# Hfx-J/SGTD

Measured on AMD Instinct MI355X. Metric: query frames/sec vs map size (descriptor build + candidate selection), higher is better.
Workload: dtype f64

## Files before the change

sgtd_amd/csrc/build_kernel.hip.h:

```cpp
#pragma once
#include "common.hip.h"

struct DescArrays {
  double *side, *angle, *center;
  float *vertex;
  int *label;
  u32 *frame;
  int *node_id;
  QueryRec *qrec;
};

#define SGTD_BUILD_THREADS 1024
#ifdef SGTD_EXP_PHASE
__device__ unsigned long long g_bphase[8];
#define BPH(i) do { if (tid == 0) { const unsigned long long _n = __builtin_readcyclecounter(); atomicAdd(&g_bphase[i], _n - bph_t); bph_t = _n; } } while (0)
#else
#define BPH(i) do { } while (0)
#endif
#define SGTD_TRI_INVALID 0xFFFFFFFFFFFFFFFFull
#define SGTD_SLOT_EMPTY 0xFFFFFFFFu

struct Tri {
  double a, b, c;
  int va, vb, vc;
  bool valid;
};

__device__ __forceinline__ double side_len(const float4 &p, const float4 &q) {
  double dx = (double)(p.x - q.x), dy = (double)(p.y - q.y), dz = (double)(p.z - q.z);
  return sqrt(dx * dx + dy * dy + dz * dz);
}

__device__ __forceinline__ Tri make_triangle(const float4 &p1, const float4 &p2,
                                             const float4 &p3, const DevCfg &cfg) {
  Tri t;
  double a = side_len(p1, p2), b = side_len(p1, p3), c = side_len(p3, p2);
  t.valid = !(a > cfg.max_len || b > cfg.max_len || c > cfg.max_len ||
              a < cfg.min_len || b < cfg.min_len || c < cfg.min_len);
  int sa = 0, sb = 1, sc = 2;
  double tmp; int ti;
  if (a > b) { tmp = a; a = b; b = tmp; ti = sa; sa = sb; sb = ti; }
  if (b > c) { tmp = b; b = c; c = tmp; ti = sb; sb = sc; sc = ti; }
  if (a > b) { tmp = a; a = b; b = tmp; ti = sa; sa = sb; sb = ti; }
  t.a = a; t.b = b; t.c = c;
  t.va = sa + sb - 1;
  t.vb = sa + sc - 1;
  t.vc = sb + sc - 1;
  return t;
}

__host__ __device__ __forceinline__ u64 pack_milli_key(u64 x, u64 y, u64 z) { return (x << 42) | (y << 21) | z; }
__device__ __forceinline__ u64 milli_key(const Tri &t) {
  float kx = (float)(t.a * 1000.0), ky = (float)(t.b * 1000.0), kz = (float)(t.c * 1000.0);
  u64 x = (u64)(long long)kx, y = (u64)(long long)ky, z = (u64)(long long)kz;
  return pack_milli_key(x, y, z);
}

struct BuildParams {
  const float *xyz;
  const u32 *label;
  const long long *kp_off;
  int n_frames;
  u32 frame_id0;
  int frame_id_step;
  long long out_stride;
  u32 *out_count;
  int max_n;
  int max_slots;
  u64 *ws_keys;
  u32 *ws_slots;
};

template <bool LDS_DEDUP, int KM>
__global__ __launch_bounds__(SGTD_BUILD_THREADS) void build_frames_kernel(
    BuildParams P, DevCfg cfg, DescArrays out) {
  extern __shared__ __align__(16) unsigned char smem[];
  const int K = cfg.K, tpi = cfg.tpi;
  const int max_t = P.max_n * tpi;
  const int max_words = (max_t + 31) / 32;
  float4 *pts = reinterpret_cast<float4 *>(smem);
  size_t off = (size_t)P.max_n * 16;
  unsigned short *knn = reinterpret_cast<unsigned short *>(smem + off);
  off += (((size_t)P.max_n * K * 2) + 15) & ~(size_t)15;
  unsigned char *mn = smem + off;
  off += (((size_t)tpi * 2) + 15) & ~(size_t)15;
  u32 *winbits = reinterpret_cast<u32 *>(smem + off);
  off += (((size_t)max_words * 4) + 15) & ~(size_t)15;
  u32 *wordpre = reinterpret_cast<u32 *>(smem + off);
  off += (((size_t)(max_words + 1) * 4) + 15) & ~(size_t)15;
  u64 *keys;
  u32 *slots;
  if (LDS_DEDUP) {
    keys = reinterpret_cast<u64 *>(smem + off);
    off += (size_t)max_t * 8;
    slots = reinterpret_cast<u32 *>(smem + off);
  } else {
    keys = P.ws_keys + (size_t)blockIdx.x * max_t;
    slots = P.ws_slots + (size_t)blockIdx.x * P.max_slots;
  }
  const int tid = threadIdx.x;

  if (tid == 0) {
    int k = 0;
    for (int m = 1; m < K - 1; m++)
      for (int n = m + 1; n < K; n++) {
        mn[2 * k] = (unsigned char)m;
        mn[2 * k + 1] = (unsigned char)n;
        k++;
      }
  }

  for (int f = blockIdx.x; f < P.n_frames; f += gridDim.x) {
    const long long kp0 = P.kp_off[f];
    const int n = (int)(P.kp_off[f + 1] - kp0);
    __syncthreads();
    if (n < K) {
      if (tid == 0) P.out_count[f] = 0;
      continue;
    }
    const int T = n * tpi;
    int nslots = 64;
    while (nslots < T + 1) nslots <<= 1;
    const int nwords = (T + 31) / 32;

#ifdef SGTD_EXP_PHASE
    unsigned long long bph_t = __builtin_readcyclecounter();
#endif
    for (int i = tid; i < n; i += SGTD_BUILD_THREADS) {
      float4 p;
      p.x = P.xyz[(kp0 + i) * 3 + 0];
      p.y = P.xyz[(kp0 + i) * 3 + 1];
      p.z = P.xyz[(kp0 + i) * 3 + 2];
      p.w = __uint_as_float(P.label[kp0 + i]);
      pts[i] = p;
    }
    for (int s = tid; s < nslots; s += SGTD_BUILD_THREADS) slots[s] = SGTD_SLOT_EMPTY;
    for (int w = tid; w < nwords; w += SGTD_BUILD_THREADS) winbits[w] = 0;
    __syncthreads();

    BPH(0);
    const int parts = (3 * K <= tpi) ? 4 : 1;
    const int per_pass = SGTD_BUILD_THREADS / parts;
    for (int i0 = 0; i0 < n; i0 += per_pass) {
      const int i = i0 + tid / parts, part = tid % parts;
      float bd[KM];
      int bi[KM];
#pragma unroll
      for (int k = 0; k < KM; k++) { bd[k] = __builtin_inff(); bi[k] = 0; }
      auto insert = [&](float cd, int cj) {
        bool lt = false;
#pragma unroll
        for (int k = 0; k < KM; k++) {
          lt = lt || (cd < bd[k]);
          float td = lt ? bd[k] : cd; int tj = lt ? bi[k] : cj;
          bd[k] = lt ? cd : bd[k]; bi[k] = lt ? cj : bi[k];
          cd = td; cj = tj;
        }
      };
      if (i < n) {
        const float4 q = pts[i];
        const int j_lo = (int)((long long)n * part / parts), j_hi = (int)((long long)n * (part + 1) / parts);
        for (int j = j_lo; j < j_hi; j++) {
          const float4 p = pts[j];
          float dx = q.x - p.x, dy = q.y - p.y, dz = q.z - p.z;
          float d = dx * dx;
          d += dy * dy;
          d += dz * dz;
          insert(d, j);
        }
        if (part > 0) {
#pragma unroll
          for (int k = 0; k < KM; k++)
            if (k < K) keys[((size_t)i * 3 + (part - 1)) * K + k] = ((u64)__float_as_uint(bd[k]) << 32) | (u32)bi[k];
        }
      }
      if (parts > 1) {
        if (!LDS_DEDUP) __threadfence_block();
        __syncthreads();
        if (i < n && part == 0) {
          for (int pk = 0; pk < 3 * K; pk++) {
            const u64 v = keys[(size_t)i * 3 * K + pk];
            insert(__uint_as_float((u32)(v >> 32)), (int)(u32)v);
          }
        }
      }
      if (i < n && part == 0) {
#pragma unroll
        for (int k = 0; k < KM; k++)
          if (k < K) knn[i * K + k] = (unsigned short)bi[k];
      }
      if (parts > 1) __syncthreads();
    }
    __syncthreads();

    BPH(1);
    for (int t = tid; t < T; t += SGTD_BUILD_THREADS) {
      const int i = t / tpi, r = t - i * tpi;
      const int m = mn[2 * r], nn = mn[2 * r + 1];
      Tri tr = make_triangle(pts[i], pts[knn[i * K + m]], pts[knn[i * K + nn]], cfg);
      keys[t] = tr.valid ? milli_key(tr) : SGTD_TRI_INVALID;
    }
    if (!LDS_DEDUP) __threadfence_block();
    __syncthreads();

    BPH(2);
    for (int t = tid; t < T; t += SGTD_BUILD_THREADS) {
      const u64 key = keys[t];
      if (key == SGTD_TRI_INVALID) continue;
      u32 h = (u32)mix64(key) & (u32)(nslots - 1);
      while (true) {
        u32 cur = atomicCAS(&slots[h], SGTD_SLOT_EMPTY, (u32)t);
        if (cur == SGTD_SLOT_EMPTY) break;
        if (keys[cur] == key) { atomicMin(&slots[h], (u32)t); break; }
        h = (h + 1) & (u32)(nslots - 1);
      }
    }
    __syncthreads();
    for (int s = tid; s < nslots; s += SGTD_BUILD_THREADS) {
      u32 v = slots[s];
      if (v != SGTD_SLOT_EMPTY) atomicOr(&winbits[v >> 5], 1u << (v & 31));
    }
    __syncthreads();
    if (tid < SGTD_WAVE) {
      u32 carry = 0;
      for (int w0 = 0; w0 < nwords; w0 += SGTD_WAVE) {
        int w = w0 + tid;
        u32 c = (w < nwords) ? __popc(winbits[w]) : 0;
        u32 inc = wave_incl_scan(c);
        if (w < nwords) wordpre[w] = carry + inc - c;
        carry += __shfl(inc, SGTD_WAVE - 1);
      }
      if (tid == 0) { wordpre[nwords] = carry; P.out_count[f] = carry; }
    }
    __syncthreads();

    BPH(3);
    const u32 frame_id = P.frame_id0 + (u32)(P.frame_id_step * f);
    for (int t = tid; t < T; t += SGTD_BUILD_THREADS) {
      const u32 word = winbits[t >> 5];
      if (!((word >> (t & 31)) & 1u)) continue;
      const u32 rank = wordpre[t >> 5] + __popc(word & ((1u << (t & 31)) - 1u));
      const int i = t / tpi, r = t - i * tpi;
      const int m = mn[2 * r], nn = mn[2 * r + 1];
      float4 p[3];
      p[0] = pts[i]; p[1] = pts[knn[i * K + m]]; p[2] = pts[knn[i * K + nn]];
      const Tri tr = make_triangle(p[0], p[1], p[2], cfg);
      const float4 A = tr.va == 0 ? p[0] : (tr.va == 1 ? p[1] : p[2]);
      const float4 B = tr.vb == 0 ? p[0] : (tr.vb == 1 ? p[1] : p[2]);
      const float4 C = tr.vc == 0 ? p[0] : (tr.vc == 1 ? p[1] : p[2]);
      const size_t o = (size_t)f * P.out_stride + rank;
      const double a = tr.a, b = tr.b, c = tr.c;
      out.side[o * 3 + 0] = cfg.scale * a;
      out.side[o * 3 + 1] = cfg.scale * b;
      out.side[o * 3 + 2] = cfg.scale * c;
      out.angle[o * 3 + 0] = fabs((b * b + c * c - a * a) / (2 * b * c));
      out.angle[o * 3 + 1] = fabs((a * a + c * c - b * b) / (2 * a * c));
      out.angle[o * 3 + 2] = fabs((a * a + b * b - c * c) / (2 * a * b));
      out.center[o * 3 + 0] = (((double)A.x + (double)B.x) + (double)C.x) / 3;
      out.center[o * 3 + 1] = (((double)A.y + (double)B.y) + (double)C.y) / 3;
      out.center[o * 3 + 2] = (((double)A.z + (double)B.z) + (double)C.z) / 3;
      out.vertex[o * 9 + 0] = A.x; out.vertex[o * 9 + 1] = A.y; out.vertex[o * 9 + 2] = A.z;
      out.vertex[o * 9 + 3] = B.x; out.vertex[o * 9 + 4] = B.y; out.vertex[o * 9 + 5] = B.z;
      out.vertex[o * 9 + 6] = C.x; out.vertex[o * 9 + 7] = C.y; out.vertex[o * 9 + 8] = C.z;
      out.label[o * 3 + 0] = (int)(double)__float_as_uint(A.w);
      out.label[o * 3 + 1] = (int)(double)__float_as_uint(B.w);
      out.label[o * 3 + 2] = (int)(double)__float_as_uint(C.w);
      out.frame[o] = frame_id;
      if (out.qrec) write_query_rec(out.qrec + o, cfg.scale * a, cfg.scale * b, cfg.scale * c, cfg.rough, frame_id);
      out.node_id[o * 3 + 0] = i; out.node_id[o * 3 + 1] = m; out.node_id[o * 3 + 2] = nn;
    }
#ifdef SGTD_EXP_PHASE
    __syncthreads();
    BPH(4);
#endif
  }
}

static inline size_t build_lds_bytes(int max_n, int K, int tpi, bool lds_dedup, int max_slots) {
  size_t max_t = (size_t)max_n * tpi, words = (max_t + 31) / 32;
  auto up = [](size_t v) { return (v + 15) & ~(size_t)15; };
  size_t b = (size_t)max_n * 16 + up((size_t)max_n * K * 2) + up((size_t)tpi * 2) +
             up(words * 4) + up((words + 1) * 4);
  if (lds_dedup) b += max_t * 8 + (size_t)max_slots * 4;
  return b;
}
```

sgtd_amd/csrc/common.hip.h:

```cpp
#pragma once
#include <hip/hip_runtime.h>
#include <stdint.h>

#define SGTD_WAVE 64
#define SGTD_MAX_K 16
#define SGTD_NCELL 27
#define SGTD_MAX_CAND 64

typedef unsigned long long u64;
typedef unsigned int u32;

struct DevCfg {
  int K;
  int tpi;
  int cand_num;
  double min_len, max_len, scale, rough;
};

__device__ __forceinline__ int lane_id() { return threadIdx.x & (SGTD_WAVE - 1); }

__device__ __forceinline__ u64 lanemask_lt() {
  return (1ull << lane_id()) - 1ull;
}

__device__ __forceinline__ double norm3(double x, double y, double z) {
  return sqrt((x * x + y * y) + z * z);
}

__host__ __device__ __forceinline__ u32 label_code(int a, int b, int c) {
  return ((u32)(a & 15) << 8) | ((u32)(b & 15) << 4) | (u32)(c & 15);
}

__host__ __device__ __forceinline__ u64 pack_key(u32 code, u32 x, u32 y, u32 z) {
  return ((u64)code << 48) | ((u64)x << 32) | ((u64)y << 16) | (u64)z;
}

__host__ __device__ __forceinline__ u64 mix64(u64 k) {
  k ^= k >> 33;
  k *= 0xff51afd7ed558ccdULL;
  k ^= k >> 33;
  k *= 0xc4ceb9fe1a85ec53ULL;
  k ^= k >> 33;
  return k;
}

__host__ __device__ __forceinline__ u32 hash_key(u64 k) {
  u32 h = (u32)k * 0x9E3779B1u ^ (u32)(k >> 32) * 0x85EBCA77u;
  h ^= h >> 15;
  h *= 0x2C1B3C6Du;
  h ^= h >> 12;
  return h;
}

struct __attribute__((aligned(16))) HotEntry {
  float s0, s1, s2;
  u32 id;
};
#define SGTD_HOT_BYTES 16
struct IdMap {
  const u32 *frame_first;
  const u32 *by_frame;
  u32 bits;
  u32 frame_lo;
};
#define SGTD_DEAD_ID 0xFFFFFFFFu
__device__ __forceinline__ u32 id_local_frame(const IdMap &m, u32 id) { return id >> m.bits; }
__device__ __forceinline__ u32 id_entry(const IdMap &m, u32 id) {
  const u32 p = m.frame_first[id >> m.bits] + (id & ((1u << m.bits) - 1u));
  return m.by_frame ? m.by_frame[p] : p;
}
#define SGTD_SENTINELS 64

#define SGTD_YSLICES 2
#define SGTD_ZSLICES 3
#define SGTD_NSUB (SGTD_YSLICES * SGTD_ZSLICES)
#define SGTD_NSLICE (SGTD_NSUB + 1)
struct __attribute__((aligned(32))) BucketDir {
  u32 start;
  u32 cum[SGTD_NSLICE];
};
static_assert(sizeof(BucketDir) == 32 && SGTD_YSLICES == 2 && SGTD_ZSLICES == 3,
              "the sweep unpacks {start, cum[0..2]} and {cum[3..6]} from the two 16-B halves of a row");
#define SGTD_NRANGE (2 * SGTD_NCELL)
#define SGTD_GROUP_ROW_BYTES 1024

struct __attribute__((aligned(64))) QueryRec {
  double q0, q1, q2;
  double thr2;
  u32 qframe;
  u32 gate;
  u32 gid;
  u32 d;
  float lo2, hi2;
  float t_up;
  u32 pad;
};

__device__ __forceinline__ double sq_threshold(double thr) {
  if (!(thr > 0.0)) return 0.0;
  double y = thr * thr;
  if (!(y > 0.0)) return y;
  if (!(y < __builtin_inf())) return y;
  while (y > 0.0 && sqrt(y) >= thr) y = __longlong_as_double(__double_as_longlong(y) - 1);
  while (true) {
    const double up = __longlong_as_double(__double_as_longlong(y) + 1);
    if (!(sqrt(up) < thr)) return up;
    y = up;
  }
}

__device__ __forceinline__ u32 gate_mask(double q0, double q1, double q2) {
  double ex[3], ey[3], ez[3];
#pragma unroll
  for (int k = 0; k < 3; k++) {
    const double dx = q0 - ((double)(int)(q0 + (double)(k - 1)) + 0.5);
    const double dy = q1 - ((double)(int)(q1 + (double)(k - 1)) + 0.5);
    const double dz = q2 - ((double)(int)(q2 + (double)(k - 1)) + 0.5);
    ex[k] = dx * dx; ey[k] = dy * dy; ez[k] = dz * dz;
  }
  u32 m = 0;
#pragma unroll
  for (int c = 0; c < 27; c++)
    if (((ex[c / 9] + ey[(c / 3) % 3]) + ez[c % 3]) < 2.25) m |= 1u << c;
  return m;
}

__device__ __forceinline__ void f32_bounds(double q0, double q1, double q2, double thr, float &lo2, float &hi2) {
  const double u = 5.9604644775390625e-08;
  const double a0 = u * (4.0 * fabs(q0) + 16.0), a1 = u * (4.0 * fabs(q1) + 16.0), a2 = u * (4.0 * fabs(q2) + 16.0);
  const double A = sqrt((a0 * a0 + a1 * a1) + a2 * a2);
  const double m = 2.0 * A + 16.0 * u * thr + 1e-12;
  const double lo = thr - m, hi = thr + m;
  float l = 0.0f;
  if (lo > 0.0) {
    const double l2 = lo * lo * (1.0 - 1e-15);
    l = (float)l2;
    if ((double)l > l2) l = __uint_as_float(__float_as_uint(l) - 1u);
  }
  const double h2 = hi * hi * (1.0 + 1e-15);
  float h = (float)h2;
  if ((double)h < h2) h = __uint_as_float(__float_as_uint(h) + 1u);
  if (!(h < __builtin_inff())) h = 3.4028234663852886e38f;
  if (!(thr > 0.0) || !(h2 == h2)) { l = 0.0f; h = 0.0f; }
  lo2 = l;
  hi2 = h;
}

__device__ __forceinline__ void write_query_rec(QueryRec *out, double s0, double s1, double s2, double rough, u32 frame) {
  const double thr = norm3(s0, s1, s2) * rough;
  float lo2, hi2;
  f32_bounds(s0, s1, s2, thr, lo2, hi2);
  double2 *qr = reinterpret_cast<double2 *>(out);
  qr[0] = make_double2(s0, s1);
  qr[1] = make_double2(s2, sq_threshold(thr));
  reinterpret_cast<uint4 *>(qr)[2] = make_uint4(frame, gate_mask(s0, s1, s2), 0u, 0u);
  const double tm = thr * (1.0 + 1e-9) + 1e-12;
  float t_up = (float)tm;
  if ((double)t_up < tm) t_up = __uint_as_float(__float_as_uint(t_up) + 1u);
  if (!(tm == tm)) t_up = __builtin_inff();
  reinterpret_cast<uint4 *>(qr)[3] = make_uint4(__float_as_uint(lo2), __float_as_uint(hi2), __float_as_uint(t_up), 0u);
}

typedef float f32x2 __attribute__((ext_vector_type(2)));

struct HashSlot {
  u64 key;
  u32 bucket;
  u32 len;
};
#define SGTD_EMPTY_KEY 0xFFFFFFFFFFFFFFFFull

__device__ __forceinline__ u32 wave_incl_scan(u32 v) {
  int x = (int)v;
  x += __builtin_amdgcn_update_dpp(0, x, 0x111, 0xf, 0xf, false);
  x += __builtin_amdgcn_update_dpp(0, x, 0x112, 0xf, 0xf, false);
  x += __builtin_amdgcn_update_dpp(0, x, 0x114, 0xf, 0xf, false);
  x += __builtin_amdgcn_update_dpp(0, x, 0x118, 0xf, 0xf, false);
  x += __builtin_amdgcn_update_dpp(0, x, 0x142, 0xa, 0xf, false);
  x += __builtin_amdgcn_update_dpp(0, x, 0x143, 0xc, 0xf, false);
  return (u32)x;
}

__device__ __forceinline__ u32 wave_sum(u32 v) {
  return (u32)__builtin_amdgcn_readlane((int)wave_incl_scan(v), SGTD_WAVE - 1);
}

__device__ __forceinline__ u32 wave_max_u32(u32 v) {
  int x = (int)v;
#define SGTD_MAX_STEP(ctrl, rows) { const u32 o = (u32)__builtin_amdgcn_update_dpp(0, x, ctrl, rows, 0xf, false); x = (int)((u32)x > o ? (u32)x : o); }
  SGTD_MAX_STEP(0x111, 0xf) SGTD_MAX_STEP(0x112, 0xf) SGTD_MAX_STEP(0x114, 0xf) SGTD_MAX_STEP(0x118, 0xf)
  SGTD_MAX_STEP(0x142, 0xa) SGTD_MAX_STEP(0x143, 0xc)
#undef SGTD_MAX_STEP
  return (u32)__builtin_amdgcn_readlane(x, SGTD_WAVE - 1);
}

template <int BITS>
__device__ __forceinline__ void wave_group_rank(u32 digit, bool valid, u32 &rank, u32 &count) {
  u64 m = __ballot(valid);
#pragma unroll
  for (int b = 0; b < BITS; b++) {
    u64 bal = __ballot((digit >> b) & 1u);
    m &= ((digit >> b) & 1u) ? bal : ~bal;
  }
  rank = __popcll(m & lanemask_lt());
  count = __popcll(m);
}
```

sgtd_amd/csrc/sgtd_accel.hip:

```cpp
#include "../../include/sgtd_accel.h"

#include <hip/hip_runtime.h>

#include <algorithm>
#include <atomic>
#include <chrono>
#include <cmath>
#include <cstdio>
#include <cstring>
#include <limits>
#include <memory>
#include <string>
#include <vector>

#include "build_kernel.hip.h"
#include "common.hip.h"
#include "table_kernels.hip.h"
#include "probe_kernels.hip.h"
#include "select_kernels.hip.h"
#include "verify_kernels.hip.h"
#include "verify_mfma.hip.h"
#include "exchange_kernels.hip.h"
#include "remove_kernels.hip.h"
#include "filter_kernels.hip.h"
// ... 144 lines not shown
  DevBuf filt_rows;
  std::vector<u64> filt_host;
  u64 filt_rows_serial = 0;
  u32 filt_rows_lo = 0, filt_rows_span = 0;
  std::vector<float> poses;
  std::vector<unsigned char> has_pose;
  u64 poses_serial = 0;
  std::shared_ptr<const PositionPrior> prior, batch_prior;
  DevBuf pos_dev, prior_dev, filt_base;
  std::vector<float4> pos_host;
  u64 pos_serial = 0;
  u32 pos_lo = 0, pos_span = 0;
  u64 filt_base_serial = 0;
  u32 filt_base_lo = 0, filt_base_span = 0;
  struct PriorKey {
    u64 prior = 0, poses = 0, filt = 0;
    u32 lo = 0, span = 0;
    int n_rows = 0;
    bool operator==(const PriorKey &o) const { return prior == o.prior && poses == o.poses && filt == o.filt && lo == o.lo && span == o.span && n_rows == o.n_rows; }
  } prior_key;
  bool prior_rows_valid = false;
  DevBuf keyA, keyB, valA, valB, hist, digit_tot, flags, bad_flag;
  std::vector<DevBuf> scan_lvl;

  DevBuf kp_off_dev, xyz_dev, label_dev, ws_keys, ws_slots, cnt_scan;
  DevBuf b_kp_off_dev, b_xyz_dev, b_label_dev;
  DescStore tmp;
  DescStore fetch;
  DevBuf fetch_idx;
  DevBuf tmp_count;

  DescStore qd;
  DevBuf q_count;
  long long q_stride = 0;
  int nq = 0;
  bool batch_valid = false, batch_synced = false;
  int last_kind = 0;
  const float *last_xyz = nullptr;
  const u32 *last_label = nullptr;
  std::vector<long long> last_kp_off;
  int last_max_n = 0;
  u32 last_qframe = 0;
  bool loop_batch = false;
  int loop_skip = 0;
  DevBuf totals;
  DevBuf cursors, list, n_visit, votes, slot_of;
  DevBuf q_M, q_P, q_pairs, q_pair_base, blk_count, rec, rec_cell, rec_dis;
  DevBuf c_pair, c_blk;
  DevBuf amb_queue;
  DevBuf n_cand, cand_frame, cand_votes, pair_off, pairs;
  DevBuf v_score, v_pose, v_inlier, v_best;
  DevBuf inl_pairs, inl_off;
  bool verify_counted = false;
  DevBuf inl_counts;
  DevBuf in_block;
  size_t frame_inl_cap = 0;
  char *frame_host = nullptr;
  size_t frame_host_bytes = 0;
  DevBuf b_in, b_out;
  char *pin_build = nullptr;
  size_t pin_build_cap = 0;
  DevBuf v_hyp64, v_hyp32, v_bound;
  DevBuf v_hypB, v_tau, v_words;
  DevBuf v_okey[2], v_oval[2];
  bool verified = false;
  DevBuf r_pose, r_rmse, r_rmse_v, r_npairs, r_moments, r_flag;
  bool refined = false;
  std::vector<std::vector<uint4>> kps;
  std::vector<unsigned char> has_kps;
  u64 kps_serial = 0, kp_dev_serial = 0;
  DevBuf kp_dev, kp_word, o_cnt, o_val, o_qxyz, o_qlabel, o_qoff;
  std::vector<uint4> kp_host;
  std::vector<u64> kp_word_host;
  int kp_dev_max = 0;
  bool overlapped = false;
  DevBuf a_pose, a_fit, a_cnt, a_val, a_mom, a_assign;
  std::vector<long long> a_qoff;
  bool aligned = false;
  int *export_packed = nullptr;
  size_t export_cap = 0;
  hipEvent_t ev_cand = nullptr, ev_export_free = nullptr;
  bool export_busy = false;
  u32 batch_serial = 0;
  bool defer_lists = false;
  bool lists_pending = false;
  bool lists_masked = false;
  const u64 *verify_keep = nullptr;
  const u64 *list_keep = nullptr;
  SelectPlan plan;
  DevBuf rough_qi, rough_entry, rough_frame, rough_cell, rough_dis;
  size_t rec_cap = (size_t)1 << 25;
  bool rec_cap_fixed = false;
  size_t pair_cap = (size_t)1 << 24;
  DevBuf n_valid, cell_rows, gid, q_prefix, group_first, n_groups;
  DevBuf pos_of_slot, rec_off, pass_pool;
  size_t pool_units = 0;
  size_t group_cap = 0;
  size_t group_cap_hook = 0;
  size_t amb_min = 65536;
  int sorted_chunk = 0;
  bool diag = false;
  int select_mode = 0;
  PinnedVec<u32> h_count, h_pair_base, h_q_M;
  PinnedVec<unsigned long long> h_q_P;
  PinnedVec<int> h_n_cand, h_cand_frame, h_cand_votes;
  PinnedVec<long long> h_pair_off;
  sgtd_stats stats{};
  char *pin = nullptr;
  size_t pin_cap = 0, pin_used = 0;
  struct PinCopy { void *dst; size_t off, bytes; };
  std::vector<PinCopy> pin_pending;
};

#include "multi.hip.h"

namespace {

#define HIPCHK(call)                                                          \
  do {                                                                        \
    hipError_t _s = (call);                                                   \
    if (_s != hipSuccess) {                                                   \
      e->err = std::string(#call) + ": " + hipGetErrorString(_s);             \
      return SGTD_ERR_HIP;                                                    \
    }                                                                         \
  } while (0)
#define CHK(call)                 \
  do {                            \
    int _r = (call);              \
    if (_r != SGTD_OK) return _r; \
  } while (0)

void stale_stages(sgtd_engine *e) { e->refined = false; e->overlapped = false; e->aligned = false; }
void new_results(sgtd_engine *e, bool verified) { e->verified = verified; stale_stages(e); }

int ensure(sgtd_engine *e, DevBuf &b, size_t bytes, bool keep = false) {
  if (bytes <= b.bytes) return SGTD_OK;
  if (b.borrowed) { e->err = "a table attached from another handle cannot grow here"; return SGTD_ERR_STATE; }
  size_t want = keep ? std::max(bytes, b.bytes + b.bytes / 2) : (b.p ? bytes + bytes / 4 : bytes);
  if (!keep && b.p) {
    HIPCHK(hipStreamSynchronize(e->stream));
    HIPCHK(hipFree(b.p));
    b.p = nullptr; b.bytes = 0;
  }
  void *np = nullptr;
  {
    const hipError_t st_ = hipMalloc(&np, want);
    if (st_ != hipSuccess) {
      (void)hipGetLastError();
      e->err = "hipMalloc of " + std::to_string(want) + " bytes: " + hipGetErrorString(st_);
      return SGTD_ERR_HIP;
    }
  }
  e->stats.device_allocs_total++;
  if (keep && b.p && b.bytes) {
    HIPCHK(hipMemcpyAsync(np, b.p, b.bytes, hipMemcpyDeviceToDevice, e->stream));
    HIPCHK(hipStreamSynchronize(e->stream));
  }
  if (b.p) HIPCHK(hipFree(b.p));
  b.p = np;
  b.bytes = want;
  return SGTD_OK;
}

int ensure_store(sgtd_engine *e, DescStore &s, size_t cap, bool keep = false) {
  if (cap <= s.cap) return SGTD_OK;
  size_t want = keep ? std::max(cap, s.cap + s.cap / 2) : cap;
  CHK(ensure(e, s.side, want * 3 * sizeof(double), keep));
  CHK(ensure(e, s.angle, want * 3 * sizeof(double), keep));
  CHK(ensure(e, s.center, want * 3 * sizeof(double), keep));
  CHK(ensure(e, s.vertex, want * 9 * sizeof(float), keep));
  CHK(ensure(e, s.label, want * 3 * sizeof(int), keep));
  CHK(ensure(e, s.frame, want * sizeof(u32), keep));
  CHK(ensure(e, s.node_id, want * 3 * sizeof(int), keep));
  if (s.with_thr2) CHK(ensure(e, s.qrec, want * sizeof(QueryRec), keep));
  s.cap = want;
  return SGTD_OK;
}

void free_buf(DevBuf &b) {
  if (b.p && !b.borrowed) (void)hipFree(b.p);
  b.p = nullptr;
  b.bytes = 0;
  b.borrowed = false;
}
void free_store(DescStore &s) {
  free_buf(s.side); free_buf(s.angle); free_buf(s.center); free_buf(s.vertex);
  free_buf(s.label); free_buf(s.frame); free_buf(s.node_id); free_buf(s.qrec);
  s.cap = 0;
}

constexpr size_t kPinMax = (size_t)1 << 20, kPinCap = (size_t)16 << 20;

int xfer_sync(sgtd_engine *e) {
  HIPCHK(hipStreamSynchronize(e->stream));
  for (const auto &c : e->pin_pending) std::memcpy(c.dst, e->pin + c.off, c.bytes);
  e->pin_pending.clear();
  e->pin_used = 0;
  return SGTD_OK;
}

struct PinScope {
  sgtd_engine *e;
  explicit PinScope(sgtd_engine *e_) : e(e_) {}
  ~PinScope() {
    if (e && !e->pin_pending.empty()) {
      (void)hipStreamSynchronize(e->stream);
      e->pin_pending.clear();
      e->pin_used = 0;
    }
  }
};

int pin_room(sgtd_engine *e, size_t bytes, size_t *off) {
  if (!e->pin) {
    void *p = nullptr;
    HIPCHK(hipHostMalloc(&p, kPinCap, hipHostMallocDefault));
    e->pin = static_cast<char *>(p);
    e->pin_cap = kPinCap;
  }
  const size_t need = (bytes + 255) & ~(size_t)255;
  if (e->pin_used + need > e->pin_cap) CHK(xfer_sync(e));
  *off = e->pin_used;
  e->pin_used += need;
  return SGTD_OK;
}

int d2h(sgtd_engine *e, void *dst, const void *src_dev, size_t bytes) {
  if (bytes == 0) return SGTD_OK;
  if (bytes > kPinMax) {
    HIPCHK(hipMemcpyAsync(dst, src_dev, bytes, hipMemcpyDeviceToHost, e->stream));
    return SGTD_OK;
  }
  size_t off;
  CHK(pin_room(e, bytes, &off));
  HIPCHK(hipMemcpyAsync(e->pin + off, src_dev, bytes, hipMemcpyDeviceToHost, e->stream));
  e->pin_pending.push_back({dst, off, bytes});
  return SGTD_OK;
}

int h2d(sgtd_engine *e, void *dst_dev, const void *src, size_t bytes) {
  if (bytes == 0) return SGTD_OK;
  if (bytes > kPinMax) {
    HIPCHK(hipMemcpyAsync(dst_dev, src, bytes, hipMemcpyHostToDevice, e->stream));
    return SGTD_OK;
  }
  size_t off;
  CHK(pin_room(e, bytes, &off));
  std::memcpy(e->pin + off, src, bytes);
  HIPCHK(hipMemcpyAsync(dst_dev, e->pin + off, bytes, hipMemcpyHostToDevice, e->stream));
  return SGTD_OK;
}

int grid_for(long long n, int threads) { return (int)((n + threads - 1) / threads); }
constexpr size_t kIndexLimit = 0xFFFFFFF0ull;
constexpr size_t kRecLimit = kIndexLimit << SGTD_REC_SHIFT;
template <class K>
size_t lds_room(K *kernel) {
  hipFuncAttributes a;
  const size_t fixed = hipFuncGetAttributes(&a, reinterpret_cast<const void *>(kernel)) == hipSuccess ? a.sharedSizeBytes : 16384;
  return std::min<size_t>(150 * 1024, 160 * 1024 - std::min<size_t>(fixed, 160 * 1024));
}

int device_scan(sgtd_engine *e, const u32 *in, u32 *out, long long n, size_t lvl = 0) {
  if (n <= 0) return SGTD_OK;
  const long long per = (long long)SGTD_SCAN_THREADS * SGTD_SCAN_ITEMS;
  const long long nb = (n + per - 1) / per;
  if (nb == 1) {
    scan_apply_kernel<<<1, SGTD_SCAN_THREADS, 0, e->stream>>>(in, out, nullptr, n);
    HIPCHK(hipGetLastError());
    return SGTD_OK;
  }
  if (e->scan_lvl.size() <= lvl) e->scan_lvl.resize(lvl + 1);
  CHK(ensure(e, e->scan_lvl[lvl], (size_t)nb * sizeof(u32)));
  u32 *sums = e->scan_lvl[lvl].as<u32>();
  scan_reduce_kernel<<<(int)nb, SGTD_SCAN_THREADS, 0, e->stream>>>(in, sums, n);
  HIPCHK(hipGetLastError());
  CHK(device_scan(e, sums, sums, nb, lvl + 1));
  sums = e->scan_lvl[lvl].as<u32>();
  scan_apply_kernel<<<(int)nb, SGTD_SCAN_THREADS, 0, e->stream>>>(in, out, sums, n);
  HIPCHK(hipGetLastError());
  return SGTD_OK;
}

constexpr int kMaxKeypoints = 65535;
bool keypoint_count_ok(long long n) { return n >= 0 && n <= kMaxKeypoints; }

int launch_build(sgtd_engine *e, const float *d_xyz, const u32 *d_label, const long long *d_kp_off,
                 int n_frames, int max_n, u32 frame_id0, int frame_step, DescArrays out,
                 long long out_stride, u32 *out_count) {
  if (n_frames <= 0) return SGTD_OK;
  if (max_n > kMaxKeypoints) return SGTD_ERR_UNSUPPORTED;
  const int K = e->dc.K, tpi = e->dc.tpi;
  long long max_t = (long long)std::max(max_n, 1) * tpi;
  int max_slots = 64;
  while (max_slots < max_t + 1) max_slots <<= 1;
  const size_t lds_limit = 160 * 1024;
  size_t lds_full = build_lds_bytes(std::max(max_n, 1), K, tpi, true, max_slots);
  size_t lds_base = build_lds_bytes(std::max(max_n, 1), K, tpi, false, max_slots);
  BuildParams P;
  P.xyz = d_xyz; P.label = d_label; P.kp_off = d_kp_off; P.n_frames = n_frames;
  P.frame_id0 = frame_id0; P.frame_id_step = frame_step; P.out_stride = out_stride;
  P.out_count = out_count; P.max_n = std::max(max_n, 1); P.max_slots = max_slots;
  P.ws_keys = nullptr; P.ws_slots = nullptr;
  if (lds_full <= lds_limit) {
    int per_cu = (int)std::max<size_t>(1, lds_limit / lds_full);
    int grid = std::min(n_frames, e->n_cus * std::min(per_cu, 4));
#define SGTD_LAUNCH_BUILD(DEDUP, KM_, LDS_)                                                                    \
  do {                                                                                                          \
    HIPCHK(hipFuncSetAttribute(reinterpret_cast<const void *>(&build_frames_kernel<DEDUP, KM_>),                \
                               hipFuncAttributeMaxDynamicSharedMemorySize, (int)(LDS_)));                       \
    build_frames_kernel<DEDUP, KM_><<<grid, SGTD_BUILD_THREADS, (LDS_), e->stream>>>(P, e->dc, out);            \
  } while (0)
#define SGTD_LAUNCH_BUILD_K(DEDUP, LDS_)                                                                        \
  do {                                                                                                          \
    if (K <= 4) SGTD_LAUNCH_BUILD(DEDUP, 4, LDS_);                                                              \
    else if (K <= 8) SGTD_LAUNCH_BUILD(DEDUP, 8, LDS_);                                                         \
    else if (K <= 10) SGTD_LAUNCH_BUILD(DEDUP, 10, LDS_);                                                       \
    else if (K <= 12) SGTD_LAUNCH_BUILD(DEDUP, 12, LDS_);                                                       \
    else SGTD_LAUNCH_BUILD(DEDUP, 16, LDS_);                                                                    \
  } while (0)
    SGTD_LAUNCH_BUILD_K(true, lds_full);
  } else if (lds_base <= lds_limit) {
    int grid = std::min(n_frames, e->n_cus * 2);
    CHK(ensure(e, e->ws_keys, (size_t)grid * max_t * sizeof(u64)));
    CHK(ensure(e, e->ws_slots, (size_t)grid * max_slots * sizeof(u32)));
    P.ws_keys = e->ws_keys.as<u64>();
    P.ws_slots = e->ws_slots.as<u32>();
    SGTD_LAUNCH_BUILD_K(false, lds_base);
#undef SGTD_LAUNCH_BUILD_K
#undef SGTD_LAUNCH_BUILD
  } else {
    return SGTD_ERR_UNSUPPORTED;
  }
  HIPCHK(hipGetLastError());
  return SGTD_OK;
}

int stage_inputs(sgtd_engine *e, const float *xyz, const u32 *label, const int64_t *kp_off,
                 int n_frames, int device_ptrs, const float **d_xyz, const u32 **d_label,
                 int *max_n, bool own_set = false) {
  DevBuf &kp_buf = own_set ? e->b_kp_off_dev : e->kp_off_dev;
  DevBuf &xyz_buf = own_set ? e->b_xyz_dev : e->xyz_dev;
  DevBuf &label_buf = own_set ? e->b_label_dev : e->label_dev;
  std::vector<long long> off(n_frames + 1);
  int mx = 0;
  for (int f = 0; f <= n_frames; f++) off[f] = kp_off[f];
  for (int f = 0; f < n_frames; f++) {
    long long n = off[f + 1] - off[f];
    if (!keypoint_count_ok(n)) return SGTD_ERR_INVALID;
    mx = std::max(mx, (int)n);
  }
  *max_n = mx;
  CHK(ensure(e, kp_buf, (size_t)(n_frames + 1) * sizeof(long long)));
  if ((size_t)(n_frames + 1) * sizeof(long long) <= kPinMax) {
    CHK(h2d(e, kp_buf.p, off.data(), (size_t)(n_frames + 1) * sizeof(long long)));
  } else {
    HIPCHK(hipMemcpyAsync(kp_buf.p, off.data(), (size_t)(n_frames + 1) * sizeof(long long), hipMemcpyHostToDevice, e->stream));
    CHK(xfer_sync(e));
  }
  const long long total = off[n_frames] - off[0];
  if (device_ptrs) {
    *d_xyz = xyz;
    *d_label = label;
  } else {
    CHK(ensure(e, xyz_buf, (size_t)std::max<long long>(total + off[0], 1) * 3 * sizeof(float)));
    CHK(ensure(e, label_buf, (size_t)std::max<long long>(total + off[0], 1) * sizeof(u32)));
    if (total > 0) {
      CHK(h2d(e, xyz_buf.as<float>() + off[0] * 3, xyz + off[0] * 3,
                            (size_t)total * 3 * sizeof(float)));
      CHK(h2d(e, label_buf.as<u32>() + off[0], label + off[0], (size_t)total * sizeof(u32)));
    }
    *d_xyz = xyz_buf.as<float>();
    *d_label = label_buf.as<u32>();
  }
  return SGTD_OK;
}

int copy_out(sgtd_engine *e, const DescStore &s, size_t first, size_t n, sgtd_desc_soa *out, size_t dst0) {
  if (n == 0) return SGTD_OK;
#define CP(field, T, w)                                                                       \
  if (out->field)                                                                             \
    CHK(d2h(e, out->field + dst0 * (w), s.field.as<T>() + first * (w),             \
                          n * (w) * sizeof(T)));
  CP(side, double, 3) CP(angle, double, 3) CP(center, double, 3) CP(vertex, float, 9)
  CP(label, int, 3) CP(frame, u32, 1) CP(node_id, int, 3)
#undef CP
  CHK(xfer_sync(e));
  return SGTD_OK;
}

int copy_in(sgtd_engine *e, DescStore &s, size_t first, size_t n, const sgtd_desc_soa *in, bool wait = true) {
  if (n == 0) return SGTD_OK;
  const DescBlockOffsets bo = desc_block_offsets(n);
  static const bool block_on = [] { const char *o = getenv("SGTD_COPY_IN_BLOCK"); return !(o && !atoi(o)); }();
  if (block_on && bo.total <= (4u << 20)) {
    size_t off;
    CHK(pin_room(e, bo.total, &off));
    const void *src[7] = {in->side, in->angle, in->center, in->vertex, in->label, in->frame, in->node_id};
    void *dst[7] = {s.side.as<double>() + first * 3, s.angle.as<double>() + first * 3, s.center.as<double>() + first * 3, s.vertex.as<float>() + first * 9,
                    s.label.as<int>() + first * 3, s.frame.as<u32>() + first, s.node_id.as<int>() + first * 3};
    const size_t bytes[7] = {n * 24, n * 24, n * 24, n * 36, n * 12, n * 4, n * 12};
    u32 present = 0;
    for (int f = 0; f < 7; f++) {
      if (src[f]) { std::memcpy(e->pin + off + bo.off[f], src[f], bytes[f]); present |= 1u << f; }
      else HIPCHK(hipMemsetAsync(dst[f], 0, bytes[f], e->stream));
    }
    CHK(ensure(e, e->in_block, bo.total));
    HIPCHK(hipMemcpyAsync(e->in_block.p, e->pin + off, bo.total, hipMemcpyHostToDevice, e->stream));
    unpack_desc_block_kernel<<<(unsigned)std::min<long long>(grid_for((long long)n * 34, 256), 512), 256, 0, e->stream>>>(e->in_block.as<unsigned char>(), (u32)n, present, s.view(),
                                                                                                                       (long long)first);
    HIPCHK(hipGetLastError());
    if (wait) CHK(xfer_sync(e));
    return SGTD_OK;
  }
#define CP(field, T, w)                                                                        \
  if (in->field)                                                                               \
    CHK(h2d(e, s.field.as<T>() + first * (w), in->field, n * (w) * sizeof(T)));               \
  else                                                                                         \
    HIPCHK(hipMemsetAsync(s.field.as<T>() + first * (w), 0, n * (w) * sizeof(T), e->stream));
  CP(side, double, 3) CP(angle, double, 3) CP(center, double, 3) CP(vertex, float, 9)
  CP(label, int, 3) CP(frame, u32, 1) CP(node_id, int, 3)
#undef CP
  if (wait) CHK(xfer_sync(e));
  return SGTD_OK;
}

void note_frames(sgtd_engine *e, u32 lo, u32 hi) {
  if (!e->have_frames) {
    e->frame_lo = lo; e->frame_hi = hi; e->have_frames = true;
  } else {
    e->frame_lo = std::min(e->frame_lo, lo);
    e->frame_hi = std::max(e->frame_hi, hi);
  }
}

template <class KeyT>
int radix_sort_pairs(sgtd_engine *e, KeyT *&kin, KeyT *&kout, u32 *&vin, u32 *&vout, long long n, int bits,
                     bool skip_const, const u32 *n_dev = nullptr) {
  const int nblocks = (int)((n + SGTD_RS_TILE - 1) / SGTD_RS_TILE);
  CHK(ensure(e, e->hist, (size_t)256 * nblocks * sizeof(u32)));
  CHK(ensure(e, e->digit_tot, 256 * sizeof(u32)));
  std::vector<u32> tot(256);
  for (int shift = 0; shift < bits; shift += 8) {
    u32 *hist = e->hist.as<u32>();
    radix_hist_kernel<KeyT><<<nblocks, SGTD_RS_THREADS, 0, e->stream>>>(kin, n, shift, hist, nblocks, n_dev);
    HIPCHK(hipGetLastError());
    if (skip_const) {
      radix_digit_totals_kernel<<<256, SGTD_SCAN_THREADS, 0, e->stream>>>(hist, nblocks, e->digit_tot.as<u32>());
      HIPCHK(hipGetLastError());
      HIPCHK(hipMemcpyAsync(tot.data(), e->digit_tot.p, 256 * sizeof(u32), hipMemcpyDeviceToHost, e->stream));
      HIPCHK(hipStreamSynchronize(e->stream));
      bool constant = false;
      for (int d = 0; d < 256; d++)
        if ((long long)tot[d] == n) constant = true;
      if (constant) continue;
    }
    CHK(device_scan(e, hist, hist, (long long)256 * nblocks));
    radix_scatter_kernel<KeyT><<<nblocks, SGTD_RS_THREADS, 0, e->stream>>>(kin, vin, kout, vout, n, shift,
                                                                       e->hist.as<u32>(), nblocks, n_dev);
    HIPCHK(hipGetLastError());
    std::swap(kin, kout);
    std::swap(vin, vout);
  }
  return SGTD_OK;
}

IdMap id_map(const sgtd_engine *e, u32 bits) {
  IdMap m;
  m.frame_first = e->frame_first.as<u32>();
  m.by_frame = e->id_by_frame ? e->by_frame.as<u32>() : nullptr;
  m.bits = bits;
  m.frame_lo = e->have_frames ? e->frame_lo : 0;
  return m;
}

int build_segment(sgtd_engine *e, sgtd_engine::Segment &S, long long g0, long long g1) {
  const long long E = g1 - g0;
  S.g0 = g0; S.g1 = g1;
  S.n_buckets = 0;
  S.hash_mask = 1023;
  S.sum_len_sq = 0.0;
  S.frame_hi = e->have_frames ? e->frame_hi : 0;
  S.built = true;
  if (E == 0) {
    CHK(ensure(e, S.hash, (size_t)1024 * sizeof(HashSlot)));
    HIPCHK(hipMemsetAsync(S.hash.p, 0xFF, (size_t)1024 * sizeof(HashSlot), e->stream));
    return SGTD_OK;
  }
  const double *side = e->tab.side.as<double>() + (size_t)g0 * 3;
  const int *label = e->tab.label.as<int>() + (size_t)g0 * 3;
  const u32 *frame = e->tab.frame.as<u32>() + (size_t)g0;
  CHK(ensure(e, e->keyA, (size_t)E * sizeof(u64)));
  CHK(ensure(e, e->keyB, (size_t)E * sizeof(u64)));
  CHK(ensure(e, e->valA, (size_t)E * sizeof(u32)));
  CHK(ensure(e, e->valB, (size_t)E * sizeof(u32)));
  CHK(ensure(e, e->bad_flag, 2 * sizeof(int)));
  HIPCHK(hipMemsetAsync(e->bad_flag.p, 0, 2 * sizeof(int), e->stream));
  make_keys_kernel<<<grid_for(E, 256), 256, 0, e->stream>>>(side, label, e->keyA.as<u64>(), e->valA.as<u32>(), E,
                                                             e->bad_flag.as<int>());
  HIPCHK(hipGetLastError());
  frame_monotone_kernel<<<grid_for(E, 256), 256, 0, e->stream>>>(frame, E, e->bad_flag.as<int>() + 1);
  HIPCHK(hipGetLastError());
  int bad[2] = {0, 0};
  HIPCHK(hipMemcpyAsync(bad, e->bad_flag.p, sizeof(bad), hipMemcpyDeviceToHost, e->stream));
  HIPCHK(hipStreamSynchronize(e->stream));
  if (bad[0]) { S.built = false; return SGTD_ERR_UNSUPPORTED; }
  const bool monotone = bad[1] == 0;

  u64 *kin = e->keyA.as<u64>(), *kout = e->keyB.as<u64>();
  u32 *vin = e->valA.as<u32>(), *vout = e->valB.as<u32>();
  CHK(ensure(e, e->slice_of, (size_t)E));
  if (!monotone) {
    frame_keys_kernel<<<grid_for(E, 256), 256, 0, e->stream>>>(frame, kin, vin, E);
    HIPCHK(hipGetLastError());
    CHK(radix_sort_pairs(e, kin, kout, vin, vout, E, 32, true));
    keys_of_order_kernel<<<grid_for(E, 256), 256, 0, e->stream>>>(side, label, vin, kin, E);
    HIPCHK(hipGetLastError());
    CHK(radix_sort_pairs(e, kin, kout, vin, vout, E, 60, true));
    slice_assign_kernel<<<grid_for(E, 256), 256, 0, e->stream>>>(kin, vin, side, frame, E, e->dc.rough, e->slice_of.as<unsigned char>());
    HIPCHK(hipGetLastError());
    kin = e->keyA.as<u64>(); kout = e->keyB.as<u64>(); vin = e->valA.as<u32>(); vout = e->valB.as<u32>();
    make_keys_kernel<<<grid_for(E, 256), 256, 0, e->stream>>>(side, label, kin, vin, E, e->bad_flag.as<int>());
    HIPCHK(hipGetLastError());
  }
  CHK(radix_sort_pairs(e, kin, kout, vin, vout, E, 60, true));
  if (monotone) {
    slice_assign_kernel<<<grid_for(E, 256), 256, 0, e->stream>>>(kin, vin, side, frame, E, e->dc.rough, e->slice_of.as<unsigned char>());
    HIPCHK(hipGetLastError());
  }
  CHK(ensure(e, e->flags, (size_t)E * sizeof(u32)));
  head_flags_kernel<<<grid_for(E, 256), 256, 0, e->stream>>>(kin, e->flags.as<u32>(), E);
  HIPCHK(hipGetLastError());
  u32 last_flag = 0, last_excl = 0;
  HIPCHK(hipMemcpyAsync(&last_flag, e->flags.as<u32>() + (E - 1), sizeof(u32), hipMemcpyDeviceToHost, e->stream));
  CHK(device_scan(e, e->flags.as<u32>(), e->flags.as<u32>(), E));
  HIPCHK(hipMemcpyAsync(&last_excl, e->flags.as<u32>() + (E - 1), sizeof(u32), hipMemcpyDeviceToHost, e->stream));
  HIPCHK(hipStreamSynchronize(e->stream));
  const u32 U = last_excl + last_flag;
  S.n_buckets = U;
  CHK(ensure(e, S.bucket_start, (size_t)(U + 1) * sizeof(u32)));
  CHK(ensure(e, S.bucket_key, (size_t)U * sizeof(u64)));
  bucket_starts_kernel<<<grid_for(E, 256), 256, 0, e->stream>>>(kin, e->flags.as<u32>(), S.bucket_start.as<u32>(),
                                                                 S.bucket_key.as<u64>(), E);
  HIPCHK(hipGetLastError());
  CHK(ensure(e, S.perm, (size_t)(E + SGTD_SENTINELS) * sizeof(u32)));
  CHK(ensure(e, S.dir, (size_t)U * sizeof(BucketDir)));
  slice_partition_kernel<<<e->n_cus * 8, 256, 0, e->stream>>>(S.bucket_start.as<u32>(), U, (u32)E, vin,
                                                               e->slice_of.as<unsigned char>(), S.perm.as<u32>(),
                                                               S.dir.as<BucketDir>());
  HIPCHK(hipGetLastError());
  HotEntry *hot = nullptr;
  if (&S == &e->seg[1]) {
    sgtd_engine::Segment &M = e->seg[0];
    const size_t m_ent = (size_t)(M.g1 - M.g0) + SGTD_SENTINELS;
    CHK(ensure(e, M.hot, (m_ent + (size_t)E + SGTD_SENTINELS) * sizeof(HotEntry), true));
    hot = M.hot.as<HotEntry>() + m_ent;
  } else {
    const size_t tail_room = e->tail_max > 0 ? 0 : (size_t)std::max<long long>(262144, E / 8) + SGTD_SENTINELS;
    CHK(ensure(e, S.hot, ((size_t)(E + SGTD_SENTINELS) + tail_room) * sizeof(HotEntry)));
    hot = S.hot.as<HotEntry>();
  }
  gather_hot_kernel<<<grid_for(E + SGTD_SENTINELS, 256), 256, 0, e->stream>>>(
      S.perm.as<u32>(), side, frame, e->id_by_frame ? e->id_of_g.as<u32>() : nullptr, id_map(e, e->id_bits), hot, E, (u32)g0);
  HIPCHK(hipGetLastError());
  u32 cap = 1024;
  while (cap < 2ull * U) cap <<= 1;
  S.hash_mask = cap - 1;
  CHK(ensure(e, S.hash, (size_t)cap * sizeof(HashSlot)));
  HIPCHK(hipMemsetAsync(S.hash.p, 0xFF, (size_t)cap * sizeof(HashSlot), e->stream));
  hash_insert_kernel<<<grid_for(U, 256), 256, 0, e->stream>>>(S.bucket_key.as<u64>(), S.bucket_start.as<u32>(), U,
                                                               (u32)E, S.hash.as<HashSlot>(), S.hash_mask);
  HIPCHK(hipGetLastError());
  CHK(ensure(e, e->sq_sum, sizeof(unsigned long long)));
  HIPCHK(hipMemsetAsync(e->sq_sum.p, 0, sizeof(unsigned long long), e->stream));
  bucket_sq_kernel<<<grid_for(U, 256), 256, 0, e->stream>>>(S.bucket_start.as<u32>(), U, (u32)E, e->sq_sum.as<unsigned long long>());
  HIPCHK(hipGetLastError());
  unsigned long long sq = 0;
  HIPCHK(hipMemcpyAsync(&sq, e->sq_sum.p, sizeof(sq), hipMemcpyDeviceToHost, e->stream));
  HIPCHK(hipStreamSynchronize(e->stream));
  S.sum_len_sq = (double)sq;
  return SGTD_OK;
}

int build_idmap(sgtd_engine *e, u32 &bits) {
  const long long E = e->n_entries;
  bits = e->id_bits ? e->id_bits : 13;
  if (E == 0 || !e->have_frames) return SGTD_OK;
  const u32 lo = e->frame_lo, span = e->frame_hi - e->frame_lo + 1;
  const u32 *frame = e->tab.frame.as<u32>();
  CHK(ensure(e, e->frame_first, (size_t)span * sizeof(u32)));
  CHK(ensure(e, e->longest, 2 * sizeof(u32)));
  HIPCHK(hipMemsetAsync(e->longest.p, 0, 2 * sizeof(u32), e->stream));
  frame_monotone_kernel<<<grid_for(E, 256), 256, 0, e->stream>>>(frame, E, reinterpret_cast<int *>(e->longest.as<u32>() + 1));
  HIPCHK(hipGetLastError());
  u32 h[2] = {0, 0};
  HIPCHK(hipMemcpyAsync(h, e->longest.p, sizeof(h), hipMemcpyDeviceToHost, e->stream));
  HIPCHK(hipStreamSynchronize(e->stream));
  e->id_by_frame = h[1] != 0;
  const u32 *key = frame;
  if (e->id_by_frame) {
    CHK(ensure(e, e->keyA, (size_t)E * sizeof(u64)));
    CHK(ensure(e, e->keyB, (size_t)E * sizeof(u64)));
    CHK(ensure(e, e->valA, (size_t)E * sizeof(u32)));
    CHK(ensure(e, e->valB, (size_t)E * sizeof(u32)));
    u64 *kin = e->keyA.as<u64>(), *kout = e->keyB.as<u64>();
    u32 *vin = e->valA.as<u32>(), *vout = e->valB.as<u32>();
    frame_keys_kernel<<<grid_for(E, 256), 256, 0, e->stream>>>(frame, kin, vin, E);
    HIPCHK(hipGetLastError());
    CHK(radix_sort_pairs(e, kin, kout, vin, vout, E, 32, true));
    CHK(ensure(e, e->by_frame, (size_t)E * sizeof(u32)));
    CHK(ensure(e, e->id_of_g, (size_t)E * sizeof(u32)));
    HIPCHK(hipMemcpyAsync(e->by_frame.p, vin, (size_t)E * sizeof(u32), hipMemcpyDeviceToDevice, e->stream));
    low_words_kernel<<<grid_for(E, 256), 256, 0, e->stream>>>(kin, E, vout);
    HIPCHK(hipGetLastError());
    key = vout;
  }
  frame_first_kernel<<<grid_for(E, 256), 256, 0, e->stream>>>(key, E, lo, e->frame_first.as<u32>());
  HIPCHK(hipGetLastError());
  frame_longest_kernel<<<grid_for(E, 256), 256, 0, e->stream>>>(key, E, lo, e->frame_first.as<u32>(), e->longest.as<u32>());
  HIPCHK(hipGetLastError());
  HIPCHK(hipMemcpyAsync(h, e->longest.p, sizeof(u32), hipMemcpyDeviceToHost, e->stream));
  HIPCHK(hipStreamSynchronize(e->stream));
  u32 need = 1;
  while (need < 32 && (1ull << need) < (unsigned long long)h[0]) need++;
  auto fits = [&](u32 b) { return b < 32 && (unsigned long long)span < (1ull << (32 - b)) - 1ull; };
  if (bits < need || !fits(bits)) {
    bits = std::max<u32>(need, 13);
    if (!fits(bits)) bits = need;
    if (!fits(bits)) {
      e->err = "a 32-bit entry id cannot hold this table's frame span and its largest frame";
      return SGTD_ERR_UNSUPPORTED;
    }
  }
  if (e->id_by_frame) {
    id_of_sorted_kernel<<<grid_for(E, 256), 256, 0, e->stream>>>(key, e->by_frame.as<u32>(), E, lo, e->frame_first.as<u32>(), bits,
                                                                 e->id_of_g.as<u32>());
    HIPCHK(hipGetLastError());
// ... 2824 lines not shown
```

Measured before the change: 187,300.

## Compact winning triangles, coalesce query-record stores via DPP, tree-merge k-NN partials

The fill phase now first compacts the surviving triangle indices into a dense LDS list, so each wave handles consecutive ranks with no idle lanes. Query records are built in registers and transposed across groups of four lanes with DPP, so each lane writes one 16-byte chunk of a contiguous record and the stores coalesce. The k-NN partial merge becomes a two-step tree reduction, replacing the serial merge of three partial lists by part 0. In exchange it adds an extra LDS pass with a barrier, plus one more barrier in the k-NN merge. Phase-timing instrumentation behind SGTD_EXP_PHASE is also added.

```diff
diff --git a/sgtd_amd/csrc/build_kernel.hip.h b/sgtd_amd/csrc/build_kernel.hip.h
--- a/sgtd_amd/csrc/build_kernel.hip.h
+++ b/sgtd_amd/csrc/build_kernel.hip.h
@@ -54,6 +54,28 @@
   float kx = (float)(t.a * 1000.0), ky = (float)(t.b * 1000.0), kz = (float)(t.c * 1000.0);
   u64 x = (u64)(long long)kx, y = (u64)(long long)ky, z = (u64)(long long)kz;
   return pack_milli_key(x, y, z);
+}
+
+template <int B>
+__device__ __forceinline__ void store_query_recs_round(QueryRec *dst, const u32 (&r)[16], int nrec, int lane) {
+  const int a = lane & 3;
+  u32 w[4];
+#pragma unroll
+  for (int j = 0; j < 4; j++) {
+    const u32 x0 = (u32)__builtin_amdgcn_update_dpp(0, (int)r[j], B * 0x55, 0xF, 0xF, false);
+    const u32 x1 = (u32)__builtin_amdgcn_update_dpp(0, (int)r[4 + j], B * 0x55, 0xF, 0xF, false);
+    const u32 x2 = (u32)__builtin_amdgcn_update_dpp(0, (int)r[8 + j], B * 0x55, 0xF, 0xF, false);
+    const u32 x3 = (u32)__builtin_amdgcn_update_dpp(0, (int)r[12 + j], B * 0x55, 0xF, 0xF, false);
+    w[j] = (a & 2) ? ((a & 1) ? x3 : x2) : ((a & 1) ? x1 : x0);
+  }
+  const int rec = (lane & ~3) + B;
+  if (rec < nrec) reinterpret_cast<uint4 *>(dst + rec)[a] = make_uint4(w[0], w[1], w[2], w[3]);
+}
+__device__ __forceinline__ void store_query_recs(QueryRec *dst, const u32 (&r)[16], int nrec, int lane) {
+  store_query_recs_round<0>(dst, r, nrec, lane);
+  store_query_recs_round<1>(dst, r, nrec, lane);
+  store_query_recs_round<2>(dst, r, nrec, lane);
+  store_query_recs_round<3>(dst, r, nrec, lane);
 }
 
 struct BuildParams {
@@ -168,19 +190,25 @@
           d += dz * dz;
           insert(d, j);
         }
-        if (part > 0) {
-#pragma unroll
-          for (int k = 0; k < KM; k++)
-            if (k < K) keys[((size_t)i * 3 + (part - 1)) * K + k] = ((u64)__float_as_uint(bd[k]) << 32) | (u32)bi[k];
-        }
       }
       if (parts > 1) {
-        if (!LDS_DEDUP) __threadfence_block();
-        __syncthreads();
-        if (i < n && part == 0) {
-          for (int pk = 0; pk < 3 * K; pk++) {
-            const u64 v = keys[(size_t)i * 3 * K + pk];
-            insert(__uint_as_float((u32)(v >> 32)), (int)(u32)v);
+#pragma nounroll
+        for (int step = 0; step < 2; step++) {
+          const bool parks = step == 0 ? (part & 1) != 0 : part == 2;
+          const bool takes = step == 0 ? (part & 1) == 0 : part == 0;
+          u64 *slot = keys + ((size_t)i * 3 + (step == 0 ? (part & 2) : 1)) * K;
+          if (i < n && parks) {
+#pragma unroll
+            for (int k = 0; k < KM; k++)
+              if (k < K) slot[k] = ((u64)__float_as_uint(bd[k]) << 32) | (u32)bi[k];
+          }
+          if (!LDS_DEDUP) __threadfence_block();
+          __syncthreads();
+          if (i < n && takes) {
+            for (int pk = 0; pk < K; pk++) {
+              const u64 v = slot[pk];
+              insert(__uint_as_float((u32)(v >> 32)), (int)(u32)v);
+            }
           }
         }
       }
@@ -233,13 +261,22 @@
       if (tid == 0) { wordpre[nwords] = carry; P.out_count[f] = carry; }
     }
     __syncthreads();
+    u32 *win_t = slots;
+    for (int t = tid; t < T; t += SGTD_BUILD_THREADS) {
+      const u32 word = winbits[t >> 5];
+      if ((word >> (t & 31)) & 1u) win_t[wordpre[t >> 5] + __popc(word & ((1u << (t & 31)) - 1u))] = (u32)t;
+    }
+    if (!LDS_DEDUP) __threadfence_block();
+    __syncthreads();
 
     BPH(3);
     const u32 frame_id = P.frame_id0 + (u32)(P.frame_id_step * f);
-    for (int t = tid; t < T; t += SGTD_BUILD_THREADS) {
-      const u32 word = winbits[t >> 5];
-      if (!((word >> (t & 31)) & 1u)) continue;
-      const u32 rank = wordpre[t >> 5] + __popc(word & ((1u << (t & 31)) - 1u));
+    const int count = (int)wordpre[nwords];
+    const int lane = tid & (SGTD_WAVE - 1);
+    for (int r0 = tid - lane; r0 < count; r0 += SGTD_BUILD_THREADS) {
+      const int rank = r0 + lane;
+      const bool live = rank < count;
+      const int t = (int)win_t[live ? rank : r0];
       const int i = t / tpi, r = t - i * tpi;
       const int m = mn[2 * r], nn = mn[2 * r + 1];
       float4 p[3];
@@ -250,24 +287,30 @@
       const float4 C = tr.vc == 0 ? p[0] : (tr.vc == 1 ? p[1] : p[2]);
       const size_t o = (size_t)f * P.out_stride + rank;
       const double a = tr.a, b = tr.b, c = tr.c;
-      out.side[o * 3 + 0] = cfg.scale * a;
-      out.side[o * 3 + 1] = cfg.scale * b;
-      out.side[o * 3 + 2] = cfg.scale * c;
-      out.angle[o * 3 + 0] = fabs((b * b + c * c - a * a) / (2 * b * c));
-      out.angle[o * 3 + 1] = fabs((a * a + c * c - b * b) / (2 * a * c));
-      out.angle[o * 3 + 2] = fabs((a * a + b * b - c * c) / (2 * a * b));
-      out.center[o * 3 + 0] = (((double)A.x + (double)B.x) + (double)C.x) / 3;
-      out.center[o * 3 + 1] = (((double)A.y + (double)B.y) + (double)C.y) / 3;
-      out.center[o * 3 + 2] = (((double)A.z + (double)B.z) + (double)C.z) / 3;
-      out.vertex[o * 9 + 0] = A.x; out.vertex[o * 9 + 1] = A.y; out.vertex[o * 9 + 2] = A.z;
-      out.vertex[o * 9 + 3] = B.x; out.vertex[o * 9 + 4] = B.y; out.vertex[o * 9 + 5] = B.z;
-      out.vertex[o * 9 + 6] = C.x; out.vertex[o * 9 + 7] = C.y; out.vertex[o * 9 + 8] = C.z;
-      out.label[o * 3 + 0] = (int)(double)__float_as_uint(A.w);
-      out.label[o * 3 + 1] = (int)(double)__float_as_uint(B.w);
-      out.label[o * 3 + 2] = (int)(double)__float_as_uint(C.w);
-      out.frame[o] = frame_id;
-      if (out.qrec) write_query_rec(out.qrec + o, cfg.scale * a, cfg.scale * b, cfg.scale * c, cfg.rough, frame_id);
-      out.node_id[o * 3 + 0] = i; out.node_id[o * 3 + 1] = m; out.node_id[o * 3 + 2] = nn;
+      if (live) {
+        out.side[o * 3 + 0] = cfg.scale * a;
+        out.side[o * 3 + 1] = cfg.scale * b;
+        out.side[o * 3 + 2] = cfg.scale * c;
+        out.angle[o * 3 + 0] = fabs((b * b + c * c - a * a) / (2 * b * c));
+        out.angle[o * 3 + 1] = fabs((a * a + c * c - b * b) / (2 * a * c));
+        out.angle[o * 3 + 2] = fabs((a * a + b * b - c * c) / (2 * a * b));
+        out.center[o * 3 + 0] = (((double)A.x + (double)B.x) + (double)C.x) / 3;
+        out.center[o * 3 + 1] = (((double)A.y + (double)B.y) + (double)C.y) / 3;
+        out.center[o * 3 + 2] = (((double)A.z + (double)B.z) + (double)C.z) / 3;
+        out.vertex[o * 9 + 0] = A.x; out.vertex[o * 9 + 1] = A.y; out.vertex[o * 9 + 2] = A.z;
+        out.vertex[o * 9 + 3] = B.x; out.vertex[o * 9 + 4] = B.y; out.vertex[o * 9 + 5] = B.z;
+        out.vertex[o * 9 + 6] = C.x; out.vertex[o * 9 + 7] = C.y; out.vertex[o * 9 + 8] = C.z;
+        out.label[o * 3 + 0] = (int)(double)__float_as_uint(A.w);
+        out.label[o * 3 + 1] = (int)(double)__float_as_uint(B.w);
+        out.label[o * 3 + 2] = (int)(double)__float_as_uint(C.w);
+        out.frame[o] = frame_id;
+        out.node_id[o * 3 + 0] = i; out.node_id[o * 3 + 1] = m; out.node_id[o * 3 + 2] = nn;
+      }
+      if (out.qrec) {
+        u32 qr[16];
+        make_query_rec(qr, cfg.scale * a, cfg.scale * b, cfg.scale * c, cfg.rough, frame_id);
+        store_query_recs(out.qrec + ((size_t)f * P.out_stride + r0), qr, count - r0, lane);
+      }
     }
 #ifdef SGTD_EXP_PHASE
     __syncthreads();
diff --git a/sgtd_amd/csrc/common.hip.h b/sgtd_amd/csrc/common.hip.h
--- a/sgtd_amd/csrc/common.hip.h
+++ b/sgtd_amd/csrc/common.hip.h
@@ -146,19 +146,29 @@
   hi2 = h;
 }
 
-__device__ __forceinline__ void write_query_rec(QueryRec *out, double s0, double s1, double s2, double rough, u32 frame) {
+__device__ __forceinline__ void make_query_rec(u32 (&r)[16], double s0, double s1, double s2, double rough, u32 frame) {
   const double thr = norm3(s0, s1, s2) * rough;
   float lo2, hi2;
   f32_bounds(s0, s1, s2, thr, lo2, hi2);
-  double2 *qr = reinterpret_cast<double2 *>(out);
-  qr[0] = make_double2(s0, s1);
-  qr[1] = make_double2(s2, sq_threshold(thr));
-  reinterpret_cast<uint4 *>(qr)[2] = make_uint4(frame, gate_mask(s0, s1, s2), 0u, 0u);
+  const double d[4] = {s0, s1, s2, sq_threshold(thr)};
+#pragma unroll
+  for (int k = 0; k < 4; k++) {
+    const unsigned long long b = (unsigned long long)__double_as_longlong(d[k]);
+    r[2 * k] = (u32)b;
+    r[2 * k + 1] = (u32)(b >> 32);
+  }
+  r[8] = frame; r[9] = gate_mask(s0, s1, s2); r[10] = 0u; r[11] = 0u;
   const double tm = thr * (1.0 + 1e-9) + 1e-12;
   float t_up = (float)tm;
   if ((double)t_up < tm) t_up = __uint_as_float(__float_as_uint(t_up) + 1u);
   if (!(tm == tm)) t_up = __builtin_inff();
-  reinterpret_cast<uint4 *>(qr)[3] = make_uint4(__float_as_uint(lo2), __float_as_uint(hi2), __float_as_uint(t_up), 0u);
+  r[12] = __float_as_uint(lo2); r[13] = __float_as_uint(hi2); r[14] = __float_as_uint(t_up); r[15] = 0u;
+}
+__device__ __forceinline__ void write_query_rec(QueryRec *out, double s0, double s1, double s2, double rough, u32 frame) {
+  u32 r[16];
+  make_query_rec(r, s0, s1, s2, rough, frame);
+#pragma unroll
+  for (int k = 0; k < 4; k++) reinterpret_cast<uint4 *>(out)[k] = make_uint4(r[4 * k], r[4 * k + 1], r[4 * k + 2], r[4 * k + 3]);
 }
 
 typedef float f32x2 __attribute__((ext_vector_type(2)));
diff --git a/sgtd_amd/csrc/sgtd_accel.hip b/sgtd_amd/csrc/sgtd_accel.hip
--- a/sgtd_amd/csrc/sgtd_accel.hip
+++ b/sgtd_amd/csrc/sgtd_accel.hip
@@ -470,6 +470,15 @@
   P.frame_id0 = frame_id0; P.frame_id_step = frame_step; P.out_stride = out_stride;
   P.out_count = out_count; P.max_n = std::max(max_n, 1); P.max_slots = max_slots;
   P.ws_keys = nullptr; P.ws_slots = nullptr;
+#ifdef SGTD_EXP_PHASE
+  static int bcalls = 0;
+  const bool bph_print = out.qrec && ++bcalls == 4;
+  unsigned long long bph0[8];
+  if (bph_print) {
+    HIPCHK(hipStreamSynchronize(e->stream));
+    HIPCHK(hipMemcpyFromSymbol(bph0, HIP_SYMBOL(g_bphase), sizeof(bph0)));
+  }
+#endif
   if (lds_full <= lds_limit) {
     int per_cu = (int)std::max<size_t>(1, lds_limit / lds_full);
     int grid = std::min(n_frames, e->n_cus * std::min(per_cu, 4));
@@ -501,6 +510,17 @@
     return SGTD_ERR_UNSUPPORTED;
   }
   HIPCHK(hipGetLastError());
+#ifdef SGTD_EXP_PHASE
+  if (bph_print) {
+    HIPCHK(hipStreamSynchronize(e->stream));
+    unsigned long long ph[8];
+    HIPCHK(hipMemcpyFromSymbol(ph, HIP_SYMBOL(g_bphase), sizeof(ph)));
+    double tot = 0;
+    for (int i = 0; i < 5; i++) { ph[i] -= bph0[i]; tot += (double)ph[i]; }
+    fprintf(stderr, "BUILD PHASE (fractions of %.0f cycles over %d frames, %.0f per frame): set-up %.3f k-NN %.3f keys %.3f dedup+prefix %.3f fill %.3f\n",
+            tot, n_frames, tot / n_frames, ph[0] / tot, ph[1] / tot, ph[2] / tot, ph[3] / tot, ph[4] / tot);
+  }
+#endif
   return SGTD_OK;
 }
 
```

Result: no change. 188,500, median of 6 (+0.7%).
